# nicolaivicol/otto-recommender

Measured on AMD Instinct MI355X. Metric: co-visit pairs/sec + candidates/sec at 220M events, 1/2/4/8 MI355X, higher is better.
Workload: dtype int32; 1 GPU; configs[1]: all 5 co-visitation rules, 220M events, 100k-session files; events=220000079, sessions=13435907, parallelism=files dealt over 1 GPU(s)

## Files before the change

### otto-recommender_amd/csrc/abi.hip

```cpp
#include <cstdarg>
#include <cstdlib>
#include <ctime>
#include <algorithm>
#include <mutex>
#include "prims.h"
#include "covis_kernels.h"
#include "table.h"

using namespace ottohip;

namespace ottohip {
static thread_local char g_err[1024] = "";
void set_error(const char* fmt, ...) {
  va_list ap;
  va_start(ap, fmt);
  vsnprintf(g_err, sizeof g_err, fmt, ap);
  va_end(ap);
}
}

namespace ottohip {
Ctx* ctx_base(ottohip_ctx* c) { return c; }

int ensure_part_stats(const ottohip_table* tc) {
// ... 182 lines not shown
  if (ev->n_files < 1 || !ev->file_session_bounds) { set_error("need >= 1 file"); return OTTOHIP_EINVAL; }
  if (ev->file_session_bounds[0] != 0 || ev->file_session_bounds[ev->n_files] != Sn) {
    set_error("file_session_bounds must start at 0 and end at n_sessions"); return OTTOHIP_EINVAL;
  }
  for (int f = 0; f < ev->n_files; ++f)
    if (ev->file_session_bounds[f + 1] < ev->file_session_bounds[f]) { set_error("file bounds not monotone"); return OTTOHIP_EINVAL; }
  if (ev->n_files > 65535) { set_error("n_files > 65535"); return OTTOHIP_ELIMIT; }
  return 0;
}

static int setup_rules(const ottohip_rule* rules, int n_rules, const ottohip_covis_params* params, int n_files_total,
                       RulesDev& R, Layout& Lt, bool allow_sym = false) {
  if (n_rules < 1 || n_rules > MAX_RULES) { set_error("n_rules=%d outside [1, %d]", n_rules, MAX_RULES); return OTTOHIP_EINVAL; }
  if (params->n_items < 1 || params->n_items > (1 << 30)) { set_error("n_items=%d outside [1, 2^30]", params->n_items); return OTTOHIP_ERANGE; }
  if (n_files_total > 65535) { set_error("n_files > 65535"); return OTTOHIP_ELIMIT; }
  memset(&R, 0, sizeof R);
  int max_per_type = 1;
  for (int r = 0; r < n_rules; ++r) {
    const ottohip_rule& q = rules[r];
    if (q.this_type < 0 || q.this_type > 2 || (q.next_type_mask & ~7u) || q.max_abs_dt < 0) {
      set_error("rule %d invalid", r); return OTTOHIP_EINVAL;
    }
    R.lo[r] = std::max(params->min_dt, -q.max_abs_dt);
    R.hi[r] = std::min(params->max_dt, q.max_abs_dt);
    R.mask[r] = q.next_type_mask;
    int t = q.this_type;
    R.rule_of_type[t][R.n_of_type[t]++] = r;
    max_per_type = std::max(max_per_type, R.n_of_type[t]);
  }
  for (int r = 0; r < n_rules; ++r)
    if (R.lo[r] > R.hi[r]) R.mask[r] = 0;
  static const bool sym_env = !(getenv("OTTOHIP_SYMMETRIC") && !strcmp(getenv("OTTOHIP_SYMMETRIC"), "0"));
  if (allow_sym && sym_env)
    for (int r = 0; r < n_rules; ++r) {
      const int t = rules[r].this_type;
      bool taken = false;
      for (int q = 0; q < r; ++q) taken |= ((R.sym_mask >> q) & 1u) && rules[q].this_type == t;
      if (!taken && R.mask[r] == (1u << t) && R.lo[r] == -R.hi[r]) R.sym_mask |= 1u << r;
    }
  Lt.A = std::max(1, bits_for((uint64_t)params->n_items));
  Lt.F = bits_for((uint64_t)n_files_total);
  Lt.BR = bits_for((uint64_t)max_per_type);
  Lt.WB = Lt.BR + Lt.A + Lt.F;
  Lt.amask = (1u << Lt.A) - 1u;
  if (Lt.WB > 31) {
    set_error("word layout %d rule + %d aid + %d file bits > 31: reduce files per call", Lt.BR, Lt.A, Lt.F);
    return OTTOHIP_ELIMIT;
  }
  return 0;
}

static ottohip_table* new_table(ottohip_ctx* ctx, int n_rules, int32_t n_items) {
  ottohip_table* T = new ottohip_table();
  T->device = ctx->device;
  T->n_rules = n_rules;
  T->n_items = n_items;
  T->ctx = ctx;
  memset(T->stats, 0, sizeof T->stats);
  return T;
}

static int owner_map(ottohip_ctx* ctx, int32_t n_items, int G, hipStream_t s, const uint32_t** a2l,
                     const uint32_t** l2a, const uint32_t** obase, int* LB) {
  uint32_t *da2l, *dl2a, *dob;
  OH_TRY(ctx->ws.get("om_a2l", (size_t)std::max(n_items, 1), &da2l));
  OH_TRY(ctx->ws.get("om_l2a", (size_t)std::max(n_items, 1), &dl2a));
  OH_TRY(ctx->ws.get("om_obase", (size_t)G + 1, &dob));
  if (ctx->om_items != n_items || ctx->om_parts != G) {
    std::vector<uint32_t> cnt(G + 1, 0), a2l_h(std::max(n_items, 1)), l2a_h(std::max(n_items, 1));
    for (int32_t a = 0; a < n_items; ++a) a2l_h[a] = cnt[owner_dev((uint32_t)a, (uint32_t)G)]++;
    uint32_t mx = 0;
    std::vector<uint32_t> ob(G + 1, 0);
    for (int o = 0; o < G; ++o) { mx = std::max(mx, cnt[o]); ob[o + 1] = ob[o] + cnt[o]; }
    for (int32_t a = 0; a < n_items; ++a) l2a_h[ob[owner_dev((uint32_t)a, (uint32_t)G)] + a2l_h[a]] = (uint32_t)a;
    OH_HIP(hipMemcpyAsync(da2l, a2l_h.data(), (size_t)n_items * 4, hipMemcpyHostToDevice, s));
    OH_HIP(hipMemcpyAsync(dl2a, l2a_h.data(), (size_t)n_items * 4, hipMemcpyHostToDevice, s));
    OH_HIP(hipMemcpyAsync(dob, ob.data(), (size_t)(G + 1) * 4, hipMemcpyHostToDevice, s));
    OH_HIP(hipStreamSynchronize(s));
    ctx->om_items = n_items;
    ctx->om_parts = G;
    ctx->om_lb = std::max(1, bits_for((uint64_t)mx));
  }
  *a2l = da2l; *l2a = dl2a; *obase = dob; *LB = ctx->om_lb;
  return 0;
}

static int covis_front(ottohip_ctx* ctx, const ottohip_events* ev, const ottohip_covis_params* params,
                       const int32_t* file_ids, int n_parts, Front& F, hipStream_t s, ottohip_emit* EM = nullptr) {
  ++ctx->gen;
  const int64_t E = ev->n_events, Sn = ev->n_sessions;
  F.E = E; F.Sn = Sn;
  F.P = 0; F.Rn = 0;
  if (E == 0 || Sn == 0) return 0;
  Workspace& ws = ctx->ws;
  const Layout& Lt = F.Lt;
  const RulesDev& R = F.R;
  const int64_t NB = ceil_div(E, EV_BLOCK);
  F.NB = NB;
  int32_t* n_long;
  int* err;
  const int64_t long_cap = E / (LCAP + 1) + 1;
  OH_TRY(ws.get("first", (size_t)NB + 1, &F.first));
  OH_TRY(ws.get("fb", (size_t)ev->n_files + 1, &F.fb));
  OH_TRY(ws.get("fid", (size_t)ev->n_files, &F.fid));
  OH_TRY(ws.get("long_list", (size_t)long_cap, &F.long_list));
  OH_TRY(ws.get("n_long", 4, &n_long));
  OH_TRY(ws.get("err", 4, &err));
  std::vector<uint32_t> fid(ev->n_files);
  for (int f = 0; f < ev->n_files; ++f) fid[f] = file_ids ? (uint32_t)file_ids[f] : (uint32_t)f;
  OH_HIP(hipMemcpyAsync(F.fb, ev->file_session_bounds, (ev->n_files + 1) * sizeof(int64_t), hipMemcpyHostToDevice, s));
  OH_HIP(hipMemcpyAsync(F.fid, fid.data(), ev->n_files * sizeof(uint32_t), hipMemcpyHostToDevice, s));
  OH_HIP(hipMemsetAsync(n_long, 0, 4 * sizeof(int32_t), s));
  OH_HIP(hipMemsetAsync(err, 0, sizeof(int), s));
  OH_HIP(hipStreamSynchronize(s));
  const int64_t* off = ev->session_offsets;
  F.off = off;

  uint32_t *rk, *pos, *rk2, *pos2;
  OH_TRY(ws.get("ev", (size_t)E, &F.evp));
  OH_TRY(ws.get("cnt", (size_t)E, &F.cnt));
  OH_TRY(ws.get("rk", (size_t)E, &rk));
  OH_TRY(ws.get("pos", (size_t)E, &pos));
  OH_TRY(ws.get("rk2", (size_t)E, &rk2));
  OH_TRY(ws.get("pos2", (size_t)E, &pos2));
  static const bool rows_legacy = getenv("OTTOHIP_ROWS") && !strcmp(getenv("OTTOHIP_ROWS"), "legacy");
  const int cshift = (Lt.A + 2 + 7) / 8 * 8;
  const bool ol_env = !(getenv("OTTOHIP_OWNER_LOCAL") && !strcmp(getenv("OTTOHIP_OWNER_LOCAL"), "0"));
  const uint32_t *om_a2l = nullptr, *om_l2a = nullptr, *om_obase = nullptr;
  int om_lb = 0;
  bool owner_local = false;
  if (!rows_legacy && n_parts > 1 && ol_env && cshift + 8 <= 32 && 3ull * (uint64_t)params->n_items < (1ull << 24)) {
    OH_TRY(owner_map(ctx, params->n_items, n_parts, s, &om_a2l, &om_l2a, &om_obase, &om_lb));
    owner_local = ((uint64_t)n_parts << (om_lb + 2)) < (1ull << cshift);
  }
  const bool fused = !rows_legacy && (n_parts == 1 || owner_local) && cshift + 8 <= 32 &&
                     3ull * (uint64_t)params->n_items < (1ull << 24);
  uint32_t* pos_w = fused ? nullptr : pos;
  static const bool rows_atomic = getenv("OTTOHIP_ROWS") && !strcmp(getenv("OTTOHIP_ROWS"), "atomic");
  const bool group = fused && !rows_atomic && !(getenv("OTTOHIP_GROUP") && !strcmp(getenv("OTTOHIP_GROUP"), "0"));
  F.link = nullptr;
  if (group) OH_TRY(ws.get("link", (size_t)E, &F.link));
  int ph = ctx->begin("prep_count", s, 9.0 * E + 8.0 * (Sn + 1) + 8.0 * E + 12.0 * E);
  k_block_first<<<grid_for(Sn + 1), 256, 0, s>>>(off, Sn, NB, F.first, F.long_list, n_long);
  k_prep_count<<<(unsigned)NB, 64, 0, s>>>(off, F.first, NB, ev->aid, ev->ts, ev->type, F.evp, params->n_items,
                                           params->dedup, err, R, Lt.A, F.cnt, rk, pos_w, fused ? cshift : 0, F.link);
  if (hipGetLastError() != hipSuccess) { set_error("k_prep_count launch failed"); return OTTOHIP_EHIP; }
  int32_t nl = 0;
  OH_TRY(d2h(&nl, n_long, 1, s));
  F.nl = nl;
  if (nl > 0) {
    std::vector<int32_t> ll(nl);
    OH_TRY(d2h(ll.data(), F.long_list, (size_t)nl, s));
    std::sort(ll.begin(), ll.end());
    OH_HIP(hipMemcpy(F.long_list, ll.data(), nl * sizeof(int32_t), hipMemcpyHostToDevice));
    std::vector<int64_t> loff(nl + 1);
    loff[0] = 0;
    for (int i = 0; i < nl; ++i) {
      int64_t ab[2];
      OH_HIP(hipMemcpy(ab, off + ll[i], 2 * sizeof(int64_t), hipMemcpyDeviceToHost));
      loff[i + 1] = loff[i] + (ab[1] - ab[0]);
    }
    OH_TRY(ws.get("long_scr", (size_t)(2 * loff[nl]), &F.lscr));
    OH_TRY(ws.get("long_pscr", (size_t)(3 * (loff[nl] + nl)), &F.lpscr));
    OH_TRY(ws.get("long_off", (size_t)(nl + 1), &F.d_loff));
    OH_HIP(hipMemcpy(F.d_loff, loff.data(), (nl + 1) * sizeof(int64_t), hipMemcpyHostToDevice));
    k_prep_long<<<nl, 64, 0, s>>>(off, F.long_list, F.d_loff, F.lscr, ev->aid, ev->ts, ev->type, F.evp,
                                  params->n_items, params->dedup, err);
    k_count_long<<<nl, 64, 0, s>>>(off, F.long_list, F.d_loff, F.lscr, F.lpscr, F.evp, R, Lt.A, F.cnt, rk, pos_w,
                                   fused ? cshift : 0, F.link);
    if (hipGetLastError() != hipSuccess) { set_error("long-session launch failed"); return OTTOHIP_EHIP; }
  }
  ctx->end(ph, s);

  ph = ctx->begin("rows", s, 0);
  if (rows_atomic && fused) {
    const uint32_t INVa = 3u << Lt.A;
    const uint32_t kmask_a = Lt.A + 2 >= 32 ? ~0u : (1u << (Lt.A + 2)) - 1u;
    const int64_t nk = (int64_t)3 << Lt.A;
    uint32_t* dcnt;
    uint64_t *doff, *tot;
    OH_TRY(ws.get("ra_cnt", (size_t)(nk * RA_SUB), &dcnt));
    OH_TRY(ws.get("ra_off", (size_t)(nk * RA_SUB), &doff));
    OH_TRY(ws.get("tot", 4, &tot));
    OH_HIP(hipMemsetAsync(dcnt, 0, (size_t)(nk * RA_SUB) * 4, s));
    k_rows_atomic<<<grid_for(E, 256 * RA_PER), 256, 0, s>>>(rk, F.cnt, E, kmask_a, INVa, dcnt, pos);
    OH_TRY(exclusive_scan_u32(ctx, dcnt, doff, nk * RA_SUB, tot, s));
    uint64_t PP = 0;
    OH_TRY(d2h(&PP, tot, 1, s));
    int herr = 0;
    OH_TRY(d2h(&herr, err, 1, s));
    if (herr) { set_error("input out of range: aid outside [0, n_items) or type outside {0,1,2}"); return OTTOHIP_ERANGE; }
    F.P = PP;
    F.Rn = nk;
    OH_TRY(ws.get("row_key", (size_t)nk, &F.row_key));
    OH_TRY(ws.get("row_begin", (size_t)nk, &F.row_begin));
    k_rows_dense<<<grid_for(nk), 256, 0, s>>>(doff, nk, F.row_key, F.row_begin);
    F.poff = nullptr; F.poff32 = nullptr;
    if (F.P < (1ull << 32)) OH_TRY(ws.get("poff32", (size_t)E, &F.poff32));
    else OH_TRY(ws.get("poff", (size_t)E, &F.poff));
    k_rows_atomic_off<<<grid_for(E, 256 * RA_PER), 256, 0, s>>>(rk, E, kmask_a, INVa, doff, pos, F.poff32, F.poff);
    OH_HIP(hipGetLastError());
    ctx->end(ph, s);
    return 0;
  }
  uint32_t INV = 3u << Lt.A;
  int kbits = Lt.A + 2;
  uint32_t kmask = Lt.A + 2 >= 32 ? ~0u : (1u << (Lt.A + 2)) - 1u;
  if (owner_local) {
    const uint32_t INV2 = (uint32_t)n_parts << (om_lb + 2);
    k_owner_key_local<<<grid_for(E), 256, 0, s>>>(rk, E, INV, Lt.A, (uint32_t)n_parts, om_lb, INV2,
                                                 (1u << cshift) - 1u, om_a2l);
    INV = INV2;
    kbits = bits_for((uint64_t)INV2 + 1);
    kmask = (1u << cshift) - 1u;
  } else if (n_parts > 1) {
    const uint32_t INV2 = (uint32_t)n_parts << (Lt.A + 2);
    k_owner_key<<<grid_for(E), 256, 0, s>>>(rk, E, INV, Lt.A, (uint32_t)n_parts, INV2);
    INV = INV2;
    kbits = Lt.A + 2 + bits_for((uint64_t)n_parts + 1);
    if (kbits > 32) { set_error("row key with owner bits > 32 bits"); return OTTOHIP_ELIMIT; }
  }
  uint32_t *rks = rk, *poss = pos;
  int64_t En = E;
  const SortSkip skip{fused ? (1u << cshift) - 1u : 0u, INV, &En};
  OH_TRY(radix_sort_pairs(ctx, rks, poss, rk2, pos2, E, kbits, s, fused, fused ? &skip : nullptr));
  uint64_t* tot;
  OH_TRY(ws.get("tot", 4, &tot));
  if (fused) {
    const uint32_t* csrc = F.link ? F.link : F.cnt;
    const int64_t nb = ceil_div(En, RT_TILE);
    uint64_t *bsum, *boff;
    OH_TRY(ws.get("rt_sums", (size_t)std::max<int64_t>(nb, 1), &bsum));
    OH_TRY(ws.get("rt_offs", (size_t)std::max<int64_t>(nb, 1), &boff));
    if (nb > 0) k_rows_sums<<<(unsigned)nb, RT_T, 0, s>>>(rks, poss, csrc, En, kmask, INV, cshift, bsum);
    OH_TRY(exclusive_scan_u64(ctx, bsum, boff, nb, tot, s));
    uint64_t X = 0;
    OH_TRY(d2h(&X, tot, 1, s));
    int herr = 0;
    OH_TRY(d2h(&herr, err, 1, s));
    if (herr) { set_error("input out of range: aid outside [0, n_items) or type outside {0,1,2}"); return OTTOHIP_ERANGE; }
    F.P = X >> 24;
    F.Rn = (int64_t)(X & 0xFFFFFFull);
    OH_TRY(ws.get("row_key", (size_t)std::max<int64_t>(F.Rn, 1), &F.row_key));
    OH_TRY(ws.get("row_begin", (size_t)std::max<int64_t>(F.Rn, 1), &F.row_begin));
    static const char* p32env = getenv("OTTOHIP_POFF32");
    F.poff = nullptr; F.poff32 = nullptr;
    if (F.P < (1ull << 32) && !(p32env && !strcmp(p32env, "0"))) {
      OH_TRY(ws.get("poff32", (size_t)E, &F.poff32));
      static const char* ppenv = getenv("OTTOHIP_POFF_PART");
      if (!(ppenv && !strcmp(ppenv, "0")) && En > 4096) {
        uint32_t* rkA = rks == rk ? rk2 : rk;
        uint32_t* posA = poss == pos ? pos2 : pos;
        k_rows_tile<<<(unsigned)nb, RT_T, 0, s>>>(rks, poss, csrc, En, kmask, INV, cshift, boff, nullptr, F.poff32, 0u,
                                                  0xFFFFFFFFu, 1, F.row_key, F.row_begin, rkA);
        const uint64_t* dstart = nullptr;
        int ntl = 0;
        OH_TRY(radix_pass(ctx, poss, rkA, posA, rks, En, std::max(0, bits_for((uint64_t)E) - 8), s, &dstart, &ntl));
        static const bool pxcd = getenv("OTTOHIP_POFF_XCD") && !strcmp(getenv("OTTOHIP_POFF_XCD"), "1");
        if (pxcd)
          k_poff_scatter_xcd<<<(unsigned)(8 * std::max(1, ctx->n_cu)), 256, 0, s>>>(posA, rks, En, dstart, ntl, F.poff32);
        else
          k_poff_scatter<<<grid_for(En), 256, 0, s>>>(posA, rks, En, F.poff32);
      } else if (nb > 0) {
        k_rows_tile<<<(unsigned)nb, RT_T, 0, s>>>(rks, poss, csrc, En, kmask, INV, cshift, boff, nullptr, F.poff32, 0u,
                                                  0xFFFFFFFFu, 1, F.row_key, F.row_begin);
      }
    } else {
      OH_TRY(ws.get("poff", (size_t)E, &F.poff));
      if (nb > 0)
        k_rows_tile<<<(unsigned)nb, RT_T, 0, s>>>(rks, poss, csrc, En, kmask, INV, cshift, boff, F.poff, nullptr, 0u, 0u,
                                                  1, F.row_key, F.row_begin);
    }
    if (F.link) k_link_fix<<<grid_for(E, 256 * LF_PER), 256, 0, s>>>(F.link, E, F.poff32, F.poff);
    if (owner_local && F.Rn > 0)
      k_rows_decode<<<grid_for(F.Rn), 256, 0, s>>>(F.row_key, F.Rn, Lt.A, om_lb, om_obase, om_l2a);
    OH_HIP(hipGetLastError());
    ctx->end(ph, s);
    return 0;
  }
  uint32_t *c_sorted = (rks == rk) ? rk2 : rk, *row_flag = (poss == pos) ? pos2 : pos;
  k_gather_counts<<<grid_for(E), 256, 0, s>>>(rks, poss, F.cnt, E, INV, c_sorted, row_flag);
  uint64_t *woff, *row_idx;
  OH_TRY(ws.get("woff", (size_t)E, &woff));
  OH_TRY(ws.get("row_idx", (size_t)E, &row_idx));
  OH_TRY(exclusive_scan_u32(ctx, c_sorted, woff, E, tot, s));
  OH_TRY(exclusive_scan_u32(ctx, row_flag, row_idx, E, tot + 1, s));
  uint64_t PR[2];
  OH_TRY(d2h(PR, tot, 2, s));
  int herr = 0;
  OH_TRY(d2h(&herr, err, 1, s));
  if (herr) { set_error("input out of range: aid outside [0, n_items) or type outside {0,1,2}"); return OTTOHIP_ERANGE; }
  F.P = PR[0];
  F.Rn = (int64_t)PR[1];
  OH_TRY(ws.get("poff", (size_t)E, &F.poff));
  F.poff32 = nullptr;
  OH_TRY(ws.get("row_key", (size_t)std::max<int64_t>(F.Rn, 1), &F.row_key));
  OH_TRY(ws.get("row_begin", (size_t)std::max<int64_t>(F.Rn, 1), &F.row_begin));
  k_rows<<<grid_for(E), 256, 0, s>>>(rks, poss, E, INV, kmask, woff, row_flag, row_idx, F.poff, F.row_key,
                                     F.row_begin);
  ctx->end(ph, s);
  return 0;
}

static int covis_emit_words(ottohip_ctx* ctx, const Front& F, const ottohip_events* ev, uint32_t* w0, hipStream_t s) {
  int ph = ctx->begin("emit", s, 8.0 * F.E + 12.0 * F.E + 4.0 * (double)F.P);
  static const int dbg0 = getenv("OTTOHIP_EMIT_DBG") ? atoi(getenv("OTTOHIP_EMIT_DBG")) : 0;
  const int dbg = dbg0;
  const bool guard = getenv("OTTOHIP_DEBUG") != nullptr;
  int* eerr;
  OH_TRY(ctx->ws.get("emit_err", 4, &eerr));
// ... 1605 lines not shown
```

### otto-recommender_amd/csrc/covis_kernels.h

```cpp
#pragma once
#include "prims.h"

namespace ottohip {

constexpr int EV_BLOCK = 256;
constexpr int LCAP = 512;
constexpr int SPLIT_MEAN = 420;
constexpr int LDS_SPLIT_MEAN = 2560;
__constant__ uint32_t c_split_mean = SPLIT_MEAN;
__constant__ uint32_t c_split_runs = 0;
__constant__ uint32_t c_split_fuse = 1;
__constant__ uint32_t c_hash_prio = 0;
__constant__ uint32_t c_lds_leaf = 0;
constexpr uint32_t W_EMPTY = 0xFFFFFFFFu;
constexpr int STAT_STRIPES = 256;
constexpr int STAT_RAW = MAX_RULES * 4;
constexpr int STAT_STRIDE = STAT_RAW + 8;

struct RulesDev {
  int32_t lo[MAX_RULES], hi[MAX_RULES];
  uint32_t mask[MAX_RULES];
  int32_t n_of_type[4];
  int32_t rule_of_type[4][MAX_RULES];
  uint32_t sym_mask;
// ... 676 lines not shown
                                                    uint32_t* __restrict__ row_key, uint64_t* __restrict__ row_begin,
                                                    uint32_t* __restrict__ wsorted = nullptr) {
  const int64_t base = (int64_t)blockIdx.x * RT_TILE + (int64_t)threadIdx.x * RT_I;
  uint64_t x[RT_I];
  uint32_t key[RT_I];
  bool st[RT_I];
  uint64_t s = 0;
#pragma unroll
  for (int i = 0; i < RT_I; ++i) {
    x[i] = 0; key[i] = INV; st[i] = false;
    if (base + i < n) x[i] = rows_x(rks, poss, cnt, base + i, kmask, INV, shift, key[i], st[i]);
    s += x[i];
  }
  __shared__ uint64_t ws[RT_T / 64];
  const uint64_t incl = wave_incl_scan64(s);
  const int w = threadIdx.x >> 6;
  if ((threadIdx.x & 63) == 63) ws[w] = incl;
  __syncthreads();
  uint64_t run = offs[blockIdx.x] + incl - s;
  for (int k = 0; k < w; ++k) run += ws[k];
#pragma unroll
  for (int i = 0; i < RT_I; ++i) {
    if (wsorted && base + i < n) wsorted[base + i] = key[i] != INV ? (uint32_t)(run >> 24) : 0u;
    if (key[i] != INV) {
      const uint64_t woff = run >> 24;
      const uint32_t ps = poss[base + i];
      if (wsorted) {
      } else if (poff32) {
        if (ps - plo < pw) poff32[ps] = (uint32_t)woff;
      } else {
        poff[ps] = woff;
      }
      if (st[i] && write_rows) {
        const uint64_t r = run & 0xFFFFFFull;
        row_key[r] = key[i];
        row_begin[r] = woff;
      }
    }
    run += x[i];
  }
}

__global__ void k_poff_scatter(const uint32_t* __restrict__ pos, const uint32_t* __restrict__ woff, int64_t n,
                               uint32_t* __restrict__ poff32) {
  const int64_t k = (int64_t)blockIdx.x * blockDim.x + threadIdx.x;
  if (k < n) poff32[pos[k]] = woff[k];
}
constexpr int LF_PER = 8;
__global__ __launch_bounds__(256) void k_link_fix(const uint32_t* __restrict__ link, int64_t n,
                                                  uint32_t* __restrict__ poff32, uint64_t* __restrict__ poff) {
  const int64_t e0 = (int64_t)blockIdx.x * (256 * LF_PER) + threadIdx.x;
  uint32_t lk[LF_PER];
#pragma unroll
  for (int j = 0; j < LF_PER; ++j) lk[j] = e0 + j * 256 < n ? link[e0 + j * 256] : LK_REP;
  uint64_t o[LF_PER];
#pragma unroll
  for (int j = 0; j < LF_PER; ++j) {
    o[j] = 0;
    if (!(lk[j] & LK_REP)) {
      const int64_t r = e0 + j * 256 + (int64_t)(lk[j] >> LK_DSHIFT) - 512;
      o[j] = poff32 ? (uint64_t)poff32[r] : poff[r];
    }
  }
#pragma unroll
  for (int j = 0; j < LF_PER; ++j)
    if (!(lk[j] & LK_REP)) {
      const int64_t e = e0 + j * 256;
      if (poff32) poff32[e] = (uint32_t)(o[j] + (lk[j] & LK_GMASK));
      else poff[e] = o[j] + (lk[j] & LK_GMASK);
    }
}
__global__ __launch_bounds__(256) void k_poff_scatter_xcd(const uint32_t* __restrict__ pos,
                                                          const uint32_t* __restrict__ woff, int64_t n,
                                                          const uint64_t* __restrict__ dstart, int ntiles,
                                                          uint32_t* __restrict__ poff32) {
  const int x = blockIdx.x & 7, j = blockIdx.x >> 3, nj = gridDim.x >> 3;
  for (int d = x; d < 256; d += 8) {
    const int64_t a = (int64_t)dstart[(int64_t)d * ntiles];
    const int64_t b = d + 1 < 256 ? (int64_t)dstart[(int64_t)(d + 1) * ntiles] : n;
    const int64_t per = (b - a + nj - 1) / nj;
    const int64_t s0 = a + (int64_t)j * per, s1 = s0 + per < b ? s0 + per : b;
    for (int64_t k = s0 + threadIdx.x; k < s1; k += 256) poff32[pos[k]] = woff[k];
  }
}

constexpr int RA_SUB = 8;
__device__ __forceinline__ uint32_t ra_sub(int64_t e) { return (uint32_t)(e >> 8) & (RA_SUB - 1); }
constexpr int RA_PER = 8;
__global__ __launch_bounds__(256) void k_rows_atomic(const uint32_t* __restrict__ rk, const uint32_t* __restrict__ cnt,
                                                     int64_t n, uint32_t kmask, uint32_t INV, uint32_t* __restrict__ dcnt,
                                                     uint32_t* __restrict__ rank) {
  const int64_t e0 = (int64_t)blockIdx.x * (256 * RA_PER) + threadIdx.x;
  uint32_t key[RA_PER], c[RA_PER], r[RA_PER];
#pragma unroll
  for (int j = 0; j < RA_PER; ++j) {
    const int64_t e = e0 + j * 256;
    key[j] = e < n ? rk[e] & kmask : INV;
    c[j] = key[j] != INV ? cnt[e] : 0u;
  }
#pragma unroll
  for (int j = 0; j < RA_PER; ++j)
    r[j] = c[j] ? atomicAdd(&dcnt[(uint64_t)key[j] * RA_SUB + ra_sub(e0 + j * 256)], c[j]) : 0u;
#pragma unroll
  for (int j = 0; j < RA_PER; ++j)
    if (e0 + j * 256 < n) rank[e0 + j * 256] = r[j];
}
__global__ __launch_bounds__(256) void k_rows_atomic_off(const uint32_t* __restrict__ rk, int64_t n, uint32_t kmask,
                                                         uint32_t INV, const uint64_t* __restrict__ doff,
                                                         const uint32_t* __restrict__ rank,
                                                         uint32_t* __restrict__ poff32, uint64_t* __restrict__ poff) {
  const int64_t e0 = (int64_t)blockIdx.x * (256 * RA_PER) + threadIdx.x;
  uint64_t o[RA_PER];
#pragma unroll
  for (int j = 0; j < RA_PER; ++j) {
    const int64_t e = e0 + j * 256;
    const uint32_t key = e < n ? rk[e] & kmask : INV;
    o[j] = key != INV ? doff[(uint64_t)key * RA_SUB + ra_sub(e)] + rank[e] : 0;
  }
#pragma unroll
  for (int j = 0; j < RA_PER; ++j) {
    const int64_t e = e0 + j * 256;
    if (e < n) { if (poff32) poff32[e] = (uint32_t)o[j]; else poff[e] = o[j]; }
  }
}
__global__ void k_rows_dense(const uint64_t* __restrict__ doff, int64_t nk, uint32_t* __restrict__ row_key,
                             uint64_t* __restrict__ row_begin) {
  const int64_t r = (int64_t)blockIdx.x * blockDim.x + threadIdx.x;
  if (r >= nk) return;
  row_key[r] = (uint32_t)r;
  row_begin[r] = doff[(uint64_t)r * RA_SUB];
}

__global__ void k_owner_key(uint32_t* __restrict__ rk, int64_t n, uint32_t INV, int A, uint32_t G, uint32_t INV2) {
  const int64_t k = (int64_t)blockIdx.x * blockDim.x + threadIdx.x;
  if (k >= n) return;
  const uint32_t key = rk[k];
  rk[k] = key == INV ? INV2 : ((owner_dev(key & ((1u << A) - 1u), G) << (A + 2)) | key);
}

__global__ void k_owner_key_local(uint32_t* __restrict__ rk, int64_t n, uint32_t INV, int A, uint32_t G, int LB,
                                  uint32_t INV2, uint32_t kmask, const uint32_t* __restrict__ a2l) {
  const int64_t k = (int64_t)blockIdx.x * blockDim.x + threadIdx.x;
  if (k >= n) return;
  const uint32_t x = rk[k], key = x & kmask, hi = x & ~kmask;
  if (key == INV) { rk[k] = hi | INV2; return; }
  const uint32_t aid = key & ((1u << A) - 1u), t = key >> A;
  rk[k] = hi | (owner_dev(aid, G) << (LB + 2)) | (t << LB) | a2l[aid];
}
__global__ void k_rows_decode(uint32_t* __restrict__ row_key, int64_t R, int A, int LB,
                              const uint32_t* __restrict__ obase, const uint32_t* __restrict__ l2a) {
  const int64_t r = (int64_t)blockIdx.x * blockDim.x + threadIdx.x;
  if (r >= R) return;
  const uint32_t k = row_key[r], o = k >> (LB + 2), t = (k >> LB) & 3u, loc = k & ((1u << LB) - 1u);
  row_key[r] = (t << A) | l2a[obase[o] + loc];
}

__global__ void k_part_bounds(const uint32_t* __restrict__ row_key, int64_t R, int A, uint32_t G,
                              uint64_t* __restrict__ first_row) {
  const int64_t r = (int64_t)blockIdx.x * blockDim.x + threadIdx.x;
  if (r > R) return;
  const int64_t prev = r == 0 ? -1 : (int64_t)owner_dev(row_key[r - 1] & ((1u << A) - 1u), G);
  const int64_t cur = r == R ? (int64_t)G : (int64_t)owner_dev(row_key[r] & ((1u << A) - 1u), G);
  for (int64_t o = prev + 1; o <= cur; ++o) first_row[o] = (uint64_t)r;
}

__global__ void k_part_words(const uint64_t* __restrict__ first_row, const uint64_t* __restrict__ row_begin, int64_t R,
// ... 2676 lines not shown
```

### otto-recommender_amd/csrc/prims.h

```cpp
#pragma once
#include "common.h"

namespace ottohip {
int exclusive_scan_u32(Ctx* ctx, const uint32_t* in, uint64_t* out, int64_t n, uint64_t* total,
                       hipStream_t s);
int exclusive_scan_u64(Ctx* ctx, const uint64_t* in, uint64_t* out, int64_t n, uint64_t* total,
                       hipStream_t s);
struct SortSkip {
  uint32_t mask, inv;
  int64_t* n_out;
};
int radix_sort_pairs(Ctx* ctx, uint32_t*& keys, uint32_t*& vals, uint32_t* keys_alt, uint32_t* vals_alt,
                     int64_t n, int bits, hipStream_t s, bool iota_vals = false, const SortSkip* skip = nullptr);
int radix_pass(Ctx* ctx, const uint32_t* kin, const uint32_t* vin, uint32_t* kout, uint32_t* vout, int64_t n,
               int shift, hipStream_t s, const uint64_t** digit_start = nullptr, int* n_tiles = nullptr);
}
```

### otto-recommender_amd/csrc/prims.hip

```cpp
#include "prims.h"

namespace ottohip {

constexpr int SCAN_T = 256, SCAN_I = 8, SCAN_TILE = SCAN_T * SCAN_I;

template <class T>
__global__ __launch_bounds__(SCAN_T) void k_block_sums(const T* __restrict__ in, int64_t n,
                                                       uint64_t* __restrict__ sums) {
  const int64_t base = (int64_t)blockIdx.x * SCAN_TILE + (int64_t)threadIdx.x * SCAN_I;
  uint64_t s = 0;
#pragma unroll
  for (int i = 0; i < SCAN_I; ++i)
    if (base + i < n) s += (uint64_t)in[base + i];
  __shared__ uint64_t ws[SCAN_T / 64];
  s = wave_incl_scan64(s);
  if ((threadIdx.x & 63) == 63) ws[threadIdx.x >> 6] = s;
  __syncthreads();
  if (threadIdx.x == 0) {
    uint64_t t = 0;
    for (int w = 0; w < SCAN_T / 64; ++w) t += ws[w];
    sums[blockIdx.x] = t;
  }
}

template <class T>
__global__ __launch_bounds__(SCAN_T) void k_scan_tile(const T* __restrict__ in, int64_t n,
                                                      uint64_t* __restrict__ out,
                                                      const uint64_t* __restrict__ offs,
                                                      uint64_t* __restrict__ total) {
  const int64_t base = (int64_t)blockIdx.x * SCAN_TILE + (int64_t)threadIdx.x * SCAN_I;
  uint64_t v[SCAN_I];
  uint64_t s = 0;
#pragma unroll
  for (int i = 0; i < SCAN_I; ++i) {
    v[i] = (base + i < n) ? (uint64_t)in[base + i] : 0;
    s += v[i];
  }
  __shared__ uint64_t ws[SCAN_T / 64];
  const uint64_t incl = wave_incl_scan64(s);
  const int w = threadIdx.x >> 6;
  if ((threadIdx.x & 63) == 63) ws[w] = incl;
  __syncthreads();
  uint64_t pre = offs ? offs[blockIdx.x] : 0;
  for (int k = 0; k < w; ++k) pre += ws[k];
  uint64_t run = pre + incl - s;
#pragma unroll
  for (int i = 0; i < SCAN_I; ++i) {
    if (base + i < n) out[base + i] = run;
    run += v[i];
  }
  if (total && threadIdx.x == SCAN_T - 1 && blockIdx.x == gridDim.x - 1) *total = run;
}

template <class T>
static int scan_rec(Ctx* ctx, const T* in, uint64_t* out, int64_t n, uint64_t* total, hipStream_t s,
                    int depth) {
  if (n <= 0) {
    if (total) OH_HIP(hipMemsetAsync(total, 0, sizeof(uint64_t), s));
    return 0;
  }
  const int64_t nb = ceil_div(n, SCAN_TILE);
  if (nb == 1) {
    k_scan_tile<T><<<1, SCAN_T, 0, s>>>(in, n, out, nullptr, total);
    OH_HIP(hipGetLastError());
    return 0;
  }
  char name[32];
  snprintf(name, sizeof name, "scan_sums%d", depth);
  uint64_t* sums;
  OH_TRY(ctx->ws.get(name, (size_t)nb, &sums));
  k_block_sums<T><<<(unsigned)nb, SCAN_T, 0, s>>>(in, n, sums);
  OH_HIP(hipGetLastError());
  OH_TRY(scan_rec<uint64_t>(ctx, sums, sums, nb, nullptr, s, depth + 1));
  k_scan_tile<T><<<(unsigned)nb, SCAN_T, 0, s>>>(in, n, out, sums, total);
  OH_HIP(hipGetLastError());
  return 0;
}

int exclusive_scan_u32(Ctx* ctx, const uint32_t* in, uint64_t* out, int64_t n, uint64_t* total,
                       hipStream_t s) {
  return scan_rec<uint32_t>(ctx, in, out, n, total, s, 0);
}
int exclusive_scan_u64(Ctx* ctx, const uint64_t* in, uint64_t* out, int64_t n, uint64_t* total,
                       hipStream_t s) {
  return scan_rec<uint64_t>(ctx, in, out, n, total, s, 0);
}

#ifndef OH_RS_R
#define OH_RS_R 16
#endif
constexpr int RS_T = 256, RS_WAVES = RS_T / 64, RS_R = OH_RS_R, RS_TILE = RS_T * RS_R;
constexpr int RS_SUB = 4, RS_BLOCK = RS_TILE * RS_SUB;

__device__ __forceinline__ int xcd_tile(int b, int nb, int xcd) {
  if (!xcd) return b;
  const int q = nb >> 3, r = nb & 7, x = b & 7;
  return x * q + min(x, r) + (b >> 3);
}

template <bool SKIP = false>
__global__ __launch_bounds__(RS_T) void k_rs_hist(const uint32_t* __restrict__ keys, int64_t n, int shift,
                                                  uint32_t* __restrict__ hist, int nb, int xcd, uint32_t smask = 0u,
                                                  uint32_t sinv = 0u) {
  const int tile = xcd_tile(blockIdx.x, nb, xcd);
  __shared__ uint32_t h[RS_WAVES][256];
  for (int i = threadIdx.x; i < RS_WAVES * 256; i += RS_T) (&h[0][0])[i] = 0;
  __syncthreads();
  const int w = threadIdx.x >> 6;
  const int64_t t0 = (int64_t)tile * RS_BLOCK;
#pragma unroll 4
  for (int r = 0; r < RS_R * RS_SUB; ++r) {
    const int64_t idx = t0 + r * RS_T + threadIdx.x;
    if constexpr (SKIP) {
      const uint32_t k = idx < n ? keys[idx] : sinv;
      if ((k & smask) != sinv) atomicAdd(&h[w][(k >> shift) & 255u], 1u);
    } else {
      lds_add_runs(h[w], idx < n ? (keys[idx] >> shift) & 255u : 0u, idx < n);
    }
  }
  __syncthreads();
  for (int d = threadIdx.x; d < 256; d += RS_T) {
    uint32_t c = 0;
    for (int k = 0; k < RS_WAVES; ++k) c += h[k][d];
    hist[(int64_t)d * nb + tile] = c;
  }
}

template <bool SKIP = false>
__global__ __launch_bounds__(RS_T) void k_rs_scatter(const uint32_t* __restrict__ kin,
                                                     const uint32_t* __restrict__ vin,
                                                     uint32_t* __restrict__ kout,
                                                     uint32_t* __restrict__ vout, int64_t n, int shift,
                                                     const uint64_t* __restrict__ gofs, int nb, int iota, int xcd,
                                                     uint32_t smask = 0u, uint32_t sinv = 0u) {
  const int tile = xcd_tile(blockIdx.x, nb, xcd);
  __shared__ uint32_t wcnt[RS_WAVES][256];
  __shared__ uint32_t bstart[256];
  __shared__ uint32_t tcnt[256];
  __shared__ uint32_t run[256];
  __shared__ uint32_t wsum[RS_WAVES];
  __shared__ uint32_t tvalid;
  __shared__ uint32_t stage_k[RS_TILE];
  __shared__ uint32_t stage_v[RS_TILE];
  const int tid = threadIdx.x, w = tid >> 6, l = tid & 63;
  run[tid] = 0;
  for (int sub = 0; sub < RS_SUB; ++sub) {
    const int64_t t0 = (int64_t)tile * RS_BLOCK + (int64_t)sub * RS_TILE;
    if (t0 >= n) break;
    for (int i = tid; i < RS_WAVES * 256; i += RS_T) (&wcnt[0][0])[i] = 0;
    __syncthreads();
    uint32_t key[RS_R], val[RS_R], rnk[RS_R];
    uint32_t vmask = 0;
#pragma unroll
    for (int r = 0; r < RS_R; ++r) {
      const int64_t idx = t0 + w * (RS_R * 64) + r * 64 + l;
      bool valid = idx < n;
      key[r] = valid ? kin[idx] : 0u;
      if constexpr (SKIP) valid = valid && (key[r] & smask) != sinv;
      vmask |= valid ? (1u << r) : 0u;
      val[r] = valid ? (iota ? (uint32_t)idx : vin[idx]) : 0u;
      const uint32_t d = (key[r] >> shift) & 255u;
      uint64_t m = __ballot(valid);
#pragma unroll
      for (int b = 0; b < 8; ++b) {
        const bool bit = (d >> b) & 1u;
        const uint64_t bb = __ballot(bit);
        m &= bit ? bb : ~bb;
      }
      const uint32_t below = mbcnt(m);
      const uint32_t old = wcnt[w][d];
      __builtin_amdgcn_wave_barrier();
      if (valid && below == 0) wcnt[w][d] = old + (uint32_t)__popcll(m);
      __builtin_amdgcn_wave_barrier();
      rnk[r] = old + below;
    }
    __syncthreads();
    {
      const int d = tid;
      uint32_t tot = 0;
#pragma unroll
      for (int k = 0; k < RS_WAVES; ++k) { uint32_t c = wcnt[k][d]; wcnt[k][d] = tot; tot += c; }
      tcnt[d] = tot;
      const uint32_t incl = wave_incl_scan(tot);
      if (l == 63) wsum[w] = incl;
      __syncthreads();
      uint32_t pre = 0;
      for (int k = 0; k < w; ++k) pre += wsum[k];
      bstart[d] = pre + incl - tot;
      if (d == 255) tvalid = pre + incl;
    }
    __syncthreads();
#pragma unroll
    for (int r = 0; r < RS_R; ++r) {
      if ((vmask >> r) & 1u) {
        const uint32_t d = (key[r] >> shift) & 255u;
        const uint32_t p = bstart[d] + wcnt[w][d] + rnk[r];
        stage_k[p] = key[r];
        stage_v[p] = val[r];
      }
    }
    __syncthreads();
    const int64_t tn = SKIP ? (int64_t)tvalid : (n - t0 < RS_TILE ? n - t0 : RS_TILE);
    for (int p = tid; p < tn; p += RS_T) {
      const uint32_t k = stage_k[p];
      const uint32_t d = (k >> shift) & 255u;
      const uint64_t dst = gofs[(int64_t)d * nb + tile] + run[d] + (uint64_t)(p - bstart[d]);
      kout[dst] = k;
      vout[dst] = stage_v[p];
    }
    __syncthreads();
    run[tid] += tcnt[tid];
  }
}

static int rs_xcd() {
  static const int v = getenv("OTTOHIP_RS_XCD") && !strcmp(getenv("OTTOHIP_RS_XCD"), "1");
  return v;
}

int radix_pass(Ctx* ctx, const uint32_t* kin, const uint32_t* vin, uint32_t* kout, uint32_t* vout, int64_t n,
               int shift, hipStream_t s, const uint64_t** digit_start, int* n_tiles) {
  if (n <= 0) return 0;
  if (n >= ((int64_t)1 << 32)) { set_error("radix_pass: n=%lld too large", (long long)n); return OTTOHIP_ELIMIT; }
  const int nb = (int)ceil_div(n, RS_BLOCK);
  uint32_t* hist; uint64_t* gofs;
  OH_TRY(ctx->ws.get("rs_hist", (size_t)nb * 256, &hist));
  OH_TRY(ctx->ws.get("rs_gofs", (size_t)nb * 256, &gofs));
  k_rs_hist<<<nb, RS_T, 0, s>>>(kin, n, shift, hist, nb, rs_xcd());
  OH_HIP(hipGetLastError());
  OH_TRY(exclusive_scan_u32(ctx, hist, gofs, (int64_t)nb * 256, nullptr, s));
  k_rs_scatter<<<nb, RS_T, 0, s>>>(kin, vin, kout, vout, n, shift, gofs, nb, 0, rs_xcd());
  OH_HIP(hipGetLastError());
  if (digit_start) *digit_start = gofs;
  if (n_tiles) *n_tiles = nb;
  return 0;
}

int radix_sort_pairs(Ctx* ctx, uint32_t*& keys, uint32_t*& vals, uint32_t* keys_alt, uint32_t* vals_alt,
                     int64_t n, int bits, hipStream_t s, bool iota_vals, const SortSkip* skip) {
  if (skip) {
    if (!iota_vals || bits <= 0) { set_error("radix_sort_pairs: skipping needs iota values and bits > 0"); return OTTOHIP_EINVAL; }
    *skip->n_out = 0;
    if (n <= 0) return 0;
  } else if (n <= 1 || bits <= 0) {
    if (iota_vals && n > 1) { set_error("radix_sort_pairs: iota values need bits > 0"); return OTTOHIP_EINVAL; }
    if (iota_vals && n == 1) OH_HIP(hipMemsetAsync(vals, 0, sizeof(uint32_t), s));
    return 0;
  }
  if (n >= ((int64_t)1 << 32)) { set_error("radix_sort_pairs: n=%lld too large", (long long)n); return OTTOHIP_ELIMIT; }
  int nb = (int)ceil_div(n, RS_BLOCK);
  uint32_t* hist; uint64_t* gofs;
  OH_TRY(ctx->ws.get("rs_hist", (size_t)nb * 256, &hist));
  OH_TRY(ctx->ws.get("rs_gofs", (size_t)nb * 256, &gofs));
  uint32_t *ka = keys, *va = vals, *kb = keys_alt, *vb = vals_alt;
  for (int shift = 0; shift < bits; shift += 8) {
    if (skip && shift == 0) {
      uint64_t* tot;
      OH_TRY(ctx->ws.get("rs_total", 1, &tot));
      k_rs_hist<true><<<nb, RS_T, 0, s>>>(ka, n, 0, hist, nb, rs_xcd(), skip->mask, skip->inv);
      OH_HIP(hipGetLastError());
      OH_TRY(exclusive_scan_u32(ctx, hist, gofs, (int64_t)nb * 256, tot, s));
      k_rs_scatter<true><<<nb, RS_T, 0, s>>>(ka, va, kb, vb, n, 0, gofs, nb, 1, rs_xcd(), skip->mask, skip->inv);
      OH_HIP(hipGetLastError());
      uint64_t kept = 0;
      OH_HIP(hipMemcpyAsync(&kept, tot, sizeof kept, hipMemcpyDeviceToHost, s));
      OH_HIP(hipStreamSynchronize(s));
      n = (int64_t)kept;
      *skip->n_out = n;
      nb = (int)ceil_div(n, RS_BLOCK);
      std::swap(ka, kb); std::swap(va, vb);
      if (n <= 1) break;
      continue;
    }
    k_rs_hist<<<nb, RS_T, 0, s>>>(ka, n, shift, hist, nb, rs_xcd());
    OH_HIP(hipGetLastError());
    OH_TRY(exclusive_scan_u32(ctx, hist, gofs, (int64_t)nb * 256, nullptr, s));
    k_rs_scatter<<<nb, RS_T, 0, s>>>(ka, va, kb, vb, n, shift, gofs, nb, iota_vals && shift == 0 ? 1 : 0, rs_xcd());
    OH_HIP(hipGetLastError());
    std::swap(ka, kb); std::swap(va, vb);
  }
  keys = ka; vals = va;
  return 0;
}

}
```

Measured before the change: 86.61 billion pairs/s.

## Replace upper radix passes with LDS-bucketed row layout after skip pass

```diff
diff --git a/otto-recommender_amd/csrc/abi.hip b/otto-recommender_amd/csrc/abi.hip
--- a/otto-recommender_amd/csrc/abi.hip
+++ b/otto-recommender_amd/csrc/abi.hip
@@ -288,6 +288,66 @@
     ctx->om_lb = std::max(1, bits_for((uint64_t)mx));
   }
   *a2l = da2l; *l2a = dl2a; *obase = dob; *LB = ctx->om_lb;
+  return 0;
+}
+
+constexpr int64_t RB_MIN_ENTRIES = 1024;
+static int rows_bucket(ottohip_ctx* ctx, Front& F, hipStream_t s, uint32_t* rks, uint32_t* poss, uint32_t* rkA,
+                       uint32_t* posA, int64_t E, int64_t En, const uint64_t* dstart, int ntl, uint32_t kmask,
+                       uint32_t INV, int cshift, const int* err, bool* taken) {
+  *taken = false;
+  Workspace& ws = ctx->ws;
+  const int nhi = (int)ceil_div((int64_t)INV, 256);
+  if (nhi > RB_HI) { set_error("rows_bucket: %d key rows > %d", nhi, RB_HI); return OTTOHIP_EINVAL; }
+  const int64_t nk = (int64_t)nhi * 256;
+  const uint32_t* csrc = F.link ? F.link : F.cnt;
+  uint64_t *sums, *x, *xs;
+  uint32_t* btot;
+  OH_TRY(ws.get("rb_sums", 257, &sums));
+  OH_TRY(ws.get("rb_tot", (size_t)nk, &btot));
+  OH_TRY(ws.get("rb_x", (size_t)nk, &x));
+  OH_TRY(ws.get("rb_xs", (size_t)nk, &xs));
+  const unsigned ntile = (unsigned)ceil_div(nhi, RB_TH);
+  k_rows_bucket_count<<<256, RB_T, 0, s>>>(rks, poss, csrc, En, dstart, ntl, kmask, cshift, nhi, btot, sums);
+  k_rows_bucket_keys<<<ntile, 256, 0, s>>>(btot, nhi, x);
+  OH_HIP(hipGetLastError());
+  OH_TRY(exclusive_scan_u64(ctx, x, xs, nk, sums + 256, s));
+  std::vector<uint64_t> h(257);
+  OH_TRY(d2h(h.data(), sums, 257, s));
+  int herr = 0;
+  OH_TRY(d2h(&herr, err, 1, s));
+  if (herr) { set_error("input out of range: aid outside [0, n_items) or type outside {0,1,2}"); return OTTOHIP_ERANGE; }
+  uint64_t words = 0;
+  for (int d = 0; d < 256; ++d) words += h[d];
+  if (words >= (1ull << 32)) return 0;
+  const uint64_t X = h[256];
+  F.P = X >> 24;
+  F.Rn = (int64_t)(X & 0xFFFFFFull);
+  OH_TRY(ws.get("row_key", (size_t)std::max<int64_t>(F.Rn, 1), &F.row_key));
+  OH_TRY(ws.get("row_begin", (size_t)std::max<int64_t>(F.Rn, 1), &F.row_begin));
+  F.poff = nullptr;
+  OH_TRY(ws.get("poff32", (size_t)E, &F.poff32));
+  uint32_t* wbase = btot;
+  k_rows_bucket_layout<<<ntile, 256, 0, s>>>(x, xs, nhi, F.row_key, F.row_begin, wbase);
+  const char *denv = getenv("OTTOHIP_ROWS_DIRECT"), *penv = getenv("OTTOHIP_ROWS_PART");
+  if (denv && !strcmp(denv, "1")) {
+    k_rows_bucket_rank<true><<<256, RB_T, 0, s>>>(rks, poss, csrc, En, dstart, ntl, kmask, cshift, nhi, wbase, F.poff32,
+                                                  nullptr);
+  } else {
+    k_rows_bucket_rank<false><<<256, RB_T, 0, s>>>(rks, poss, csrc, En, dstart, ntl, kmask, cshift, nhi, wbase, nullptr,
+                                                   rkA);
+    if (penv && !strcmp(penv, "1")) {
+      OH_TRY(radix_pass(ctx, poss, rkA, posA, rks, En, std::max(0, bits_for((uint64_t)E) - 8), s));
+      k_poff_scatter<<<grid_for(En), 256, 0, s>>>(posA, rks, En, F.poff32);
+    } else {
+      constexpr int gt = PL_EV / RADIX_TILE_KEYS;
+      static_assert(gt >= 1, "an LDS image holds at least one sort tile of events");
+      k_poff_scatter_lds<<<(unsigned)ceil_div(ntl, gt), PL_T, 0, s>>>(poss, rkA, En, dstart, ntl, gt, RADIX_TILE_KEYS, E,
+                                                                    F.poff32);
+    }
+  }
+  OH_HIP(hipGetLastError());
+  *taken = true;
   return 0;
 }
 
@@ -429,9 +489,29 @@
   uint32_t *rks = rk, *poss = pos;
   int64_t En = E;
   const SortSkip skip{fused ? (1u << cshift) - 1u : 0u, INV, &En};
-  OH_TRY(radix_sort_pairs(ctx, rks, poss, rk2, pos2, E, kbits, s, fused, fused ? &skip : nullptr));
+  const char* rows_env = getenv("OTTOHIP_ROWS");
+  const char* p32_env = getenv("OTTOHIP_POFF32");
+  bool bucketed = false;
+  if (fused && n_parts == 1 && kbits <= 23 && !(rows_env && !strcmp(rows_env, "sort")) &&
+      !(p32_env && !strcmp(p32_env, "0"))) {
+    const uint64_t* dstart = nullptr;
+    int ntl = 0;
+    OH_TRY(radix_skip_pass(ctx, rk, rk2, pos2, E, s, skip, &dstart, &ntl));
+    rks = rk2; poss = pos2;
+    if (En > RB_MIN_ENTRIES)
+      OH_TRY(rows_bucket(ctx, F, s, rk2, pos2, rk, pos, E, En, dstart, ntl, kmask, INV, cshift, err, &bucketed));
+    if (!bucketed) OH_TRY(radix_sort_pairs(ctx, rks, poss, rk, pos, En, kbits, s, false, nullptr, 8));
+  } else {
+    OH_TRY(radix_sort_pairs(ctx, rks, poss, rk2, pos2, E, kbits, s, fused, fused ? &skip : nullptr));
+  }
   uint64_t* tot;
   OH_TRY(ws.get("tot", 4, &tot));
+  if (bucketed) {
+    if (F.link) k_link_fix<<<grid_for(E, 256 * LF_PER), 256, 0, s>>>(F.link, E, F.poff32, F.poff);
+    OH_HIP(hipGetLastError());
+    ctx->end(ph, s);
+    return 0;
+  }
   if (fused) {
     const uint32_t* csrc = F.link ? F.link : F.cnt;
     const int64_t nb = ceil_div(En, RT_TILE);
diff --git a/otto-recommender_amd/csrc/covis_kernels.h b/otto-recommender_amd/csrc/covis_kernels.h
--- a/otto-recommender_amd/csrc/covis_kernels.h
+++ b/otto-recommender_amd/csrc/covis_kernels.h
@@ -782,6 +782,180 @@
     const int64_t s0 = a + (int64_t)j * per, s1 = s0 + per < b ? s0 + per : b;
     for (int64_t k = s0 + threadIdx.x; k < s1; k += 256) poff32[pos[k]] = woff[k];
   }
+}
+
+constexpr int RB_T = 1024, RB_U = 8, RB_HI = 1 << 15, RB_TH = 32;
+
+__device__ __forceinline__ void rows_bucket_range(const uint64_t* __restrict__ dstart, int ntiles, int64_t n, int d,
+                                                  int64_t& a, int64_t& b) {
+  a = (int64_t)dstart[(int64_t)d * ntiles];
+  b = d + 1 < 256 ? (int64_t)dstart[(int64_t)(d + 1) * ntiles] : n;
+}
+
+__device__ __forceinline__ uint32_t rows_bucket_entry(uint32_t kk, const uint32_t* __restrict__ poss,
+                                                      const uint32_t* __restrict__ cnt, int64_t k, uint32_t kmask,
+                                                      int shift, int nhi, uint32_t& hi) {
+  hi = (kk & kmask) >> 8;
+  if (hi >= (uint32_t)nhi) { hi = 0; return 0u; }
+  uint32_t c = kk >> shift;
+  if (c == RK_CSAT) c = cnt[poss[k]] & ~LK_REP;
+  return c;
+}
+
+__global__ __launch_bounds__(RB_T) void k_rows_bucket_count(const uint32_t* __restrict__ rks,
+                                                            const uint32_t* __restrict__ poss,
+                                                            const uint32_t* __restrict__ cnt, int64_t n,
+                                                            const uint64_t* __restrict__ dstart, int ntiles,
+                                                            uint32_t kmask, int shift, int nhi,
+                                                            uint32_t* __restrict__ btot,
+                                                            uint64_t* __restrict__ bsum) {
+  __shared__ uint32_t tab[RB_HI];
+  __shared__ uint64_t ws[RB_T / 64];
+  const int d = blockIdx.x;
+  for (int i = threadIdx.x; i < nhi; i += RB_T) tab[i] = 0u;
+  __syncthreads();
+  int64_t a, b;
+  rows_bucket_range(dstart, ntiles, n, d, a, b);
+  uint64_t s = 0;
+  for (int64_t k0 = a + threadIdx.x; k0 < b; k0 += RB_T * RB_U) {
+    uint32_t kk[RB_U];
+#pragma unroll
+    for (int j = 0; j < RB_U; ++j) kk[j] = k0 + j * RB_T < b ? rks[k0 + j * RB_T] : 0u;
+#pragma unroll
+    for (int j = 0; j < RB_U; ++j) {
+      const int64_t k = k0 + j * RB_T;
+      if (k < b) {
+        uint32_t hi;
+        const uint32_t c = rows_bucket_entry(kk[j], poss, cnt, k, kmask, shift, nhi, hi);
+        if (c) atomicAdd(&tab[hi], c);
+        s += c;
+      }
+    }
+  }
+  __syncthreads();
+  for (int i = threadIdx.x; i < nhi; i += RB_T) btot[(int64_t)d * nhi + i] = tab[i];
+  s = wave_sum64(s);
+  if ((threadIdx.x & 63) == 0) ws[threadIdx.x >> 6] = s;
+  __syncthreads();
+  if (threadIdx.x == 0) {
+    uint64_t t = 0;
+    for (int w = 0; w < RB_T / 64; ++w) t += ws[w];
+    bsum[d] = t;
+  }
+}
+
+__global__ __launch_bounds__(256) void k_rows_bucket_keys(const uint32_t* __restrict__ btot, int nhi,
+                                                          uint64_t* __restrict__ x) {
+  __shared__ uint32_t t[256][RB_TH + 1];
+  const int h0 = blockIdx.x * RB_TH, hl = threadIdx.x & (RB_TH - 1);
+  for (int d = threadIdx.x / RB_TH; d < 256; d += 256 / RB_TH)
+    t[d][hl] = h0 + hl < nhi ? btot[(int64_t)d * nhi + h0 + hl] : 0u;
+  __syncthreads();
+  for (int i = 0; i < RB_TH && h0 + i < nhi; ++i) {
+    const uint32_t c = t[threadIdx.x][i];
+    x[(int64_t)(h0 + i) * 256 + threadIdx.x] = ((uint64_t)c << 24) | (c ? 1u : 0u);
+  }
+}
+
+__global__ __launch_bounds__(256) void k_rows_bucket_layout(const uint64_t* __restrict__ x,
+                                                            const uint64_t* __restrict__ xs, int nhi,
+                                                            uint32_t* __restrict__ row_key,
+                                                            uint64_t* __restrict__ row_begin,
+                                                            uint32_t* __restrict__ wbase) {
+  __shared__ uint32_t t[256][RB_TH + 1];
+  const int h0 = blockIdx.x * RB_TH, hl = threadIdx.x & (RB_TH - 1);
+  for (int i = 0; i < RB_TH && h0 + i < nhi; ++i) {
+    const int64_t k = (int64_t)(h0 + i) * 256 + threadIdx.x;
+    const uint64_t v = xs[k];
+    if (x[k] & 1u) {
+      const uint64_t r = v & 0xFFFFFFull;
+      row_key[r] = (uint32_t)k;
+      row_begin[r] = v >> 24;
+    }
+    t[threadIdx.x][i] = (uint32_t)(v >> 24);
+  }
+  __syncthreads();
+  if (h0 + hl < nhi)
+    for (int d = threadIdx.x / RB_TH; d < 256; d += 256 / RB_TH) wbase[(int64_t)d * nhi + h0 + hl] = t[d][hl];
+}
+
+template <bool DIRECT>
+__global__ __launch_bounds__(RB_T) void k_rows_bucket_rank(const uint32_t* __restrict__ rks,
+                                                           const uint32_t* __restrict__ poss,
+                                                           const uint32_t* __restrict__ cnt, int64_t n,
+                                                           const uint64_t* __restrict__ dstart, int ntiles,
+                                                           uint32_t kmask, int shift, int nhi,
+                                                           const uint32_t* __restrict__ wbase,
+                                                           uint32_t* __restrict__ poff32,
+                                                           uint32_t* __restrict__ woff) {
+  __shared__ uint32_t tab[RB_HI];
+  const int d = blockIdx.x;
+  for (int i = threadIdx.x; i < nhi; i += RB_T) tab[i] = wbase[(int64_t)d * nhi + i];
+  __syncthreads();
+  int64_t a, b;
+  rows_bucket_range(dstart, ntiles, n, d, a, b);
+  for (int64_t k0 = a + threadIdx.x; k0 < b; k0 += RB_T * RB_U) {
+    uint32_t kk[RB_U], ps[RB_U];
+#pragma unroll
+    for (int j = 0; j < RB_U; ++j) {
+      const bool in = k0 + j * RB_T < b;
+      kk[j] = in ? rks[k0 + j * RB_T] : 0u;
+      if constexpr (DIRECT) ps[j] = in ? poss[k0 + j * RB_T] : 0u;
+    }
+#pragma unroll
+    for (int j = 0; j < RB_U; ++j) {
+      const int64_t k = k0 + j * RB_T;
+      if (k < b) {
+        uint32_t hi;
+        const uint32_t c = rows_bucket_entry(kk[j], poss, cnt, k, kmask, shift, nhi, hi);
+        const uint32_t off = c ? atomicAdd(&tab[hi], c) : 0u;
+        if constexpr (DIRECT) poff32[ps[j]] = off;
+        else woff[k] = off;
+      }
+    }
+  }
+}
+
+constexpr int PL_T = 1024, PL_EV = 32768, PL_J = 4;
+__global__ __launch_bounds__(PL_T) void k_poff_scatter_lds(const uint32_t* __restrict__ pos,
+                                                           const uint32_t* __restrict__ woff, int64_t n,
+                                                           const uint64_t* __restrict__ dstart, int ntiles, int gt,
+                                                           int tile_ev, int64_t E, uint32_t* __restrict__ poff32) {
+  __shared__ uint32_t img[PL_EV];
+  const int t0 = blockIdx.x * gt, t1 = t0 + gt;
+  const int64_t p0 = (int64_t)t0 * tile_ev;
+  const uint32_t np = (uint32_t)(E - p0 < (int64_t)gt * tile_ev ? E - p0 : (int64_t)gt * tile_ev);
+  for (uint32_t i = threadIdx.x; i < np; i += PL_T) img[i] = 0u;
+  __syncthreads();
+  const int w = threadIdx.x >> 6, l = threadIdx.x & 63;
+  for (int d0 = w * (256 / (PL_T / 64)); d0 < (w + 1) * (256 / (PL_T / 64)); d0 += PL_J) {
+    int64_t k[PL_J], b[PL_J];
+#pragma unroll
+    for (int j = 0; j < PL_J; ++j) {
+      const int d = d0 + j;
+      k[j] = (int64_t)dstart[(int64_t)d * ntiles + t0] + l;
+      b[j] = t1 < ntiles ? (int64_t)dstart[(int64_t)d * ntiles + t1]
+                         : (d + 1 < 256 ? (int64_t)dstart[(int64_t)(d + 1) * ntiles] : n);
+    }
+    bool more = true;
+    while (more) {
+      uint32_t p[PL_J], o[PL_J];
+#pragma unroll
+      for (int j = 0; j < PL_J; ++j) {
+        p[j] = k[j] < b[j] ? pos[k[j]] - (uint32_t)p0 : 0xFFFFFFFFu;
+        o[j] = k[j] < b[j] ? woff[k[j]] : 0u;
+      }
+      more = false;
+#pragma unroll
+      for (int j = 0; j < PL_J; ++j) {
+        if (p[j] < np) img[p[j]] = o[j];
+        k[j] += 64;
+        more |= k[j] - l < b[j];
+      }
+    }
+  }
+  __syncthreads();
+  for (uint32_t i = threadIdx.x; i < np; i += PL_T) poff32[p0 + i] = img[i];
 }
 
 constexpr int RA_SUB = 8;
diff --git a/otto-recommender_amd/csrc/prims.h b/otto-recommender_amd/csrc/prims.h
--- a/otto-recommender_amd/csrc/prims.h
+++ b/otto-recommender_amd/csrc/prims.h
@@ -11,7 +11,14 @@
   int64_t* n_out;
 };
 int radix_sort_pairs(Ctx* ctx, uint32_t*& keys, uint32_t*& vals, uint32_t* keys_alt, uint32_t* vals_alt,
-                     int64_t n, int bits, hipStream_t s, bool iota_vals = false, const SortSkip* skip = nullptr);
+                     int64_t n, int bits, hipStream_t s, bool iota_vals = false, const SortSkip* skip = nullptr,
+                     int shift0 = 0);
+int radix_skip_pass(Ctx* ctx, const uint32_t* keys, uint32_t* kout, uint32_t* vout, int64_t n, hipStream_t s,
+                    const SortSkip& skip, const uint64_t** digit_start = nullptr, int* n_tiles = nullptr);
+#ifndef OH_RS_R
+#define OH_RS_R 16
+#endif
+constexpr int RADIX_TILE_KEYS = 256 * OH_RS_R * 4;
 int radix_pass(Ctx* ctx, const uint32_t* kin, const uint32_t* vin, uint32_t* kout, uint32_t* vout, int64_t n,
                int shift, hipStream_t s, const uint64_t** digit_start = nullptr, int* n_tiles = nullptr);
 }
diff --git a/otto-recommender_amd/csrc/prims.hip b/otto-recommender_amd/csrc/prims.hip
--- a/otto-recommender_amd/csrc/prims.hip
+++ b/otto-recommender_amd/csrc/prims.hip
@@ -86,11 +86,9 @@
   return scan_rec<uint64_t>(ctx, in, out, n, total, s, 0);
 }
 
-#ifndef OH_RS_R
-#define OH_RS_R 16
-#endif
 constexpr int RS_T = 256, RS_WAVES = RS_T / 64, RS_R = OH_RS_R, RS_TILE = RS_T * RS_R;
 constexpr int RS_SUB = 4, RS_BLOCK = RS_TILE * RS_SUB;
+static_assert(RS_BLOCK == RADIX_TILE_KEYS, "prims.h: RADIX_TILE_KEYS");
 
 __device__ __forceinline__ int xcd_tile(int b, int nb, int xcd) {
   if (!xcd) return b;
@@ -236,42 +234,58 @@
   return 0;
 }
 
+int radix_skip_pass(Ctx* ctx, const uint32_t* keys, uint32_t* kout, uint32_t* vout, int64_t n, hipStream_t s,
+                    const SortSkip& skip, const uint64_t** digit_start, int* n_tiles) {
+  *skip.n_out = 0;
+  if (n <= 0) return 0;
+  if (n >= ((int64_t)1 << 32)) { set_error("radix_skip_pass: n=%lld too large", (long long)n); return OTTOHIP_ELIMIT; }
+  const int nb = (int)ceil_div(n, RS_BLOCK);
+  uint32_t* hist; uint64_t* gofs; uint64_t* tot;
+  OH_TRY(ctx->ws.get("rs_hist", (size_t)nb * 256, &hist));
+  OH_TRY(ctx->ws.get("rs_gofs", (size_t)nb * 256, &gofs));
+  OH_TRY(ctx->ws.get("rs_total", 1, &tot));
+  k_rs_hist<true><<<nb, RS_T, 0, s>>>(keys, n, 0, hist, nb, rs_xcd(), skip.mask, skip.inv);
+  OH_HIP(hipGetLastError());
+  OH_TRY(exclusive_scan_u32(ctx, hist, gofs, (int64_t)nb * 256, tot, s));
+  k_rs_scatter<true><<<nb, RS_T, 0, s>>>(keys, nullptr, kout, vout, n, 0, gofs, nb, 1, rs_xcd(), skip.mask, skip.inv);
+  OH_HIP(hipGetLastError());
+  uint64_t kept = 0;
+  OH_HIP(hipMemcpyAsync(&kept, tot, sizeof kept, hipMemcpyDeviceToHost, s));
+  OH_HIP(hipStreamSynchronize(s));
+  *skip.n_out = (int64_t)kept;
+  if (digit_start) *digit_start = gofs;
+  if (n_tiles) *n_tiles = nb;
+  return 0;
+}
+
 int radix_sort_pairs(Ctx* ctx, uint32_t*& keys, uint32_t*& vals, uint32_t* keys_alt, uint32_t* vals_alt,
-                     int64_t n, int bits, hipStream_t s, bool iota_vals, const SortSkip* skip) {
+                     int64_t n, int bits, hipStream_t s, bool iota_vals, const SortSkip* skip, int shift0) {
   if (skip) {
-    if (!iota_vals || bits <= 0) { set_error("radix_sort_pairs: skipping needs iota values and bits > 0"); return OTTOHIP_EINVAL; }
+    if (!iota_vals || bits <= 0 || shift0 != 0) {
+      set_error("radix_sort_pairs: skipping needs iota values, bits > 0 and all digits");
+      return OTTOHIP_EINVAL;
+    }
     *skip->n_out = 0;
     if (n <= 0) return 0;
-  } else if (n <= 1 || bits <= 0) {
+    OH_TRY(radix_skip_pass(ctx, keys, keys_alt, vals_alt, n, s, *skip));
+    std::swap(keys, keys_alt); std::swap(vals, vals_alt);
+    n = *skip->n_out;
+    shift0 = 8;
+    iota_vals = false;
+  }
+  if (n <= 1 || bits <= shift0) {
     if (iota_vals && n > 1) { set_error("radix_sort_pairs: iota values need bits > 0"); return OTTOHIP_EINVAL; }
     if (iota_vals && n == 1) OH_HIP(hipMemsetAsync(vals, 0, sizeof(uint32_t), s));
     return 0;
   }
+  if (iota_vals && shift0 != 0) { set_error("radix_sort_pairs: iota values need the first digit"); return OTTOHIP_EINVAL; }
   if (n >= ((int64_t)1 << 32)) { set_error("radix_sort_pairs: n=%lld too large", (long long)n); return OTTOHIP_ELIMIT; }
-  int nb = (int)ceil_div(n, RS_BLOCK);
+  const int nb = (int)ceil_div(n, RS_BLOCK);
   uint32_t* hist; uint64_t* gofs;
   OH_TRY(ctx->ws.get("rs_hist", (size_t)nb * 256, &hist));
   OH_TRY(ctx->ws.get("rs_gofs", (size_t)nb * 256, &gofs));
   uint32_t *ka = keys, *va = vals, *kb = keys_alt, *vb = vals_alt;
-  for (int shift = 0; shift < bits; shift += 8) {
-    if (skip && shift == 0) {
-      uint64_t* tot;
-      OH_TRY(ctx->ws.get("rs_total", 1, &tot));
-      k_rs_hist<true><<<nb, RS_T, 0, s>>>(ka, n, 0, hist, nb, rs_xcd(), skip->mask, skip->inv);
-      OH_HIP(hipGetLastError());
-      OH_TRY(exclusive_scan_u32(ctx, hist, gofs, (int64_t)nb * 256, tot, s));
-      k_rs_scatter<true><<<nb, RS_T, 0, s>>>(ka, va, kb, vb, n, 0, gofs, nb, 1, rs_xcd(), skip->mask, skip->inv);
-      OH_HIP(hipGetLastError());
-      uint64_t kept = 0;
-      OH_HIP(hipMemcpyAsync(&kept, tot, sizeof kept, hipMemcpyDeviceToHost, s));
-      OH_HIP(hipStreamSynchronize(s));
-      n = (int64_t)kept;
-      *skip->n_out = n;
-      nb = (int)ceil_div(n, RS_BLOCK);
-      std::swap(ka, kb); std::swap(va, vb);
-      if (n <= 1) break;
-      continue;
-    }
+  for (int shift = shift0; shift < bits; shift += 8) {
     k_rs_hist<<<nb, RS_T, 0, s>>>(ka, n, shift, hist, nb, rs_xcd());
     OH_HIP(hipGetLastError());
     OH_TRY(exclusive_scan_u32(ctx, hist, gofs, (int64_t)nb * 256, nullptr, s));
```

Result: faster. 95.95 billion pairs/s (median of 6 runs) (+10.8%).
